# ghazalehnt/RecBole

Hardware: AMD Instinct MI355X
Metric: train positives/sec (+neg) per node (higher is better)
Workload: dtype fp32; 1 GPU; C2 BPR-MF ml-20m-shape: 138,494 users x 26,745 items (incl. PAD), ~20M interactions RO_RS 0.8/0.1/0.1, embedding 128, 4 uniform negatives, 512 positives (2,048 rows) per step, dense Adam; global_batch=512, per_gpu_batch=512, train_interactions=16014928, parallelism=single, exchange_graph=True, sampler=walk (bit-exact)

## Files before the change

include/mirec.h:

```cpp
#ifndef MIREC_H
#define MIREC_H

#include <stddef.h>
#include <stdint.h>

#ifdef __cplusplus
extern "C" {
#endif

#define MIREC_ABI_VERSION 19

int mirec_abi_version(void);
const char* mirec_last_error(void);

size_t mirec_sample_walk_workspace_size(int64_t batch_keys, int64_t num);
int mirec_sample_walk(const int32_t* random_list, int64_t L, int64_t* pr_dev,
                      const int64_t* keys, int64_t n_keys, int64_t batch_keys,
                      int64_t n_batches, int64_t num,
                      const int64_t* used_ptr, const int32_t* used_cols,
                      const uint32_t* used_bits, int64_t n_bits,
                      int64_t n_key_space, int reject,
                      int64_t* out, int64_t out_stride, int32_t* status_dev,
                      void* ws, size_t ws_bytes, void* stream);

// ... 202 lines not shown

int mirec_adam_multi_f32(const mirec_adam_table* tables, int32_t n_tables, int32_t d,
                         const float* step_consts_dev, const int32_t* step_base_dev,
                         int32_t step_off, double beta1, double beta2, double eps,
                         double weight_decay, void* stream);

#define MIREC_ADAM_ZERO_STATE 0x7fffffff
int mirec_adam_deferred_f32(const mirec_adam_table* tables, int32_t n_tables,
                            const int64_t* n_max_uniq, int32_t d,
                            const float* step_consts_dev, const int32_t* step_base_dev,
                            int32_t step_off, double beta1, double beta2, double eps,
                            double weight_decay, void* stream);
int mirec_adam_deferred_pair_f32(const mirec_adam_table* tables, const int64_t* n_max_uniq,
                                 int32_t d, const float* step_consts_dev,
                                 const int32_t* step_base_dev, int32_t step_off, double beta1,
                                 double beta2, double eps, double weight_decay, void* stream);

int mirec_adam_flush_f32(const mirec_adam_table* tables, int32_t n_tables, int32_t d,
                         const float* step_consts_dev, const int32_t* step_base_dev,
                         int32_t step_off, double beta1, double beta2, double eps,
                         double weight_decay, void* stream);
int mirec_adam_flush_rows_f32(const mirec_adam_table* tables, int32_t n_tables, int32_t d,
                              const int32_t* rows_per_wave, const float* step_consts_dev,
                              const int32_t* step_base_dev, int32_t step_off, double beta1,
                              double beta2, double eps, double weight_decay, void* stream);
int mirec_adam_flush_masked_f32(const mirec_adam_table* tables, int32_t n_tables, int32_t d,
                                const uint32_t* const* masks, const int32_t* want,
                                const int32_t* rows_per_wave, int32_t walk_waves,
                                const float* step_consts_dev, const int32_t* step_base_dev,
                                int32_t step_off, double beta1, double beta2, double eps,
                                double weight_decay, void* stream);
int mirec_row_bitmap(const int64_t* keys, int64_t n_keys, int64_t n_rows, uint32_t* bitmap,
                     void* stream);
int mirec_bpr_adam_step_f32(const mirec_adam_table* tables, const int64_t* n_max_uniq,
                            int32_t d, const int64_t* items, int64_t Bc, int32_t T, float gamma,
                            float grad_scale, float* loss_k, const int32_t* u_rec,
                            const int32_t* u_crec, const int32_t* i_rec, const int32_t* i_crec,
                            float* u_part, int32_t* u_join, float* i_part, int32_t* i_join,
                            const float* step_consts_dev, const int32_t* step_base_dev,
                            int32_t step_off, double beta1, double beta2, double eps,
                            double weight_decay, void* stream);
int mirec_step_records(const int64_t* user_keys, const int64_t* item_keys, int64_t n_batches,
                       int64_t Bc, int32_t T, int64_t n_users, int64_t n_items,
                       const int32_t* u_perm, const int32_t* u_uniq, const int32_t* u_seg,
                       const int32_t* u_nu, const int32_t* i_perm, const int32_t* i_uniq,
                       const int32_t* i_seg, const int32_t* i_nu, int32_t* u_rec,
                       int32_t* u_crec, int32_t* i_rec, int32_t* i_crec, int32_t* u_ahead,
                       int32_t* u_nah, int32_t* i_ahead, int32_t* i_nah, void* stream);
int64_t mirec_step_record_ints(int64_t per);

int mirec_copy_many(const void* const* src, void* const* dst, const int64_t* bytes, int n,
                    void* stream);

int mirec_write_bytes(void* dst_dev, const void* src_host, size_t n_bytes, void* stream);

int mirec_selftest_adam_math(uint64_t sqrt_stride, uint64_t n_div, uint64_t seed,
                             unsigned long long* out4_dev, void* stream);

int mirec_step_finish(const float* loss_k, int64_t n, float denom, float* loss_hist,
                      int32_t* step_idx_dev, void* stream);

int mirec_chunk_finish(const float* loss_k, int64_t n, int64_t stride, int32_t n_steps,
                       float denom, float* loss_hist, int32_t* step_base_dev,
                       int32_t* ticket_dev, void* stream);

int mirec_fullsort_topk_f32(const float* Uq, int64_t nq, const float* EI, int64_t I,
// ... 243 lines not shown
```

recbole_amd/_native.py:

```python
from __future__ import annotations

import ctypes
import os
from ctypes import c_double, c_float, c_int, c_int32, c_int64, c_size_t, c_void_p, c_char_p

import torch

_HERE = os.path.dirname(os.path.abspath(__file__))
LIB_PATH = os.environ.get("MIREC_LIB", os.path.join(_HERE, "_lib", "libmirec.so"))

_P = c_void_p


class RowsRef(ctypes.Structure):
    _fields_ = [('lo', _P), ('hi', _P), ('split', c_int64)]


class SpmmEpilogue(ctypes.Structure):
    _fields_ = [('add', RowsRef), ('add_scale', c_float), ('y', RowsRef), ('acc_in', RowsRef),
                ('acc_out', RowsRef), ('acc_scale', c_float)]


class CtxField(ctypes.Structure):
    _fields_ = [('kind', c_int32), ('seq_len', c_int32), ('ids', _P), ('vals', _P),
# ... 138 lines not shown
    "mirec_segment_reduce2_f32": (c_int, [_P, c_int32, _P, _P, _P, _P, _P, c_int64, _P, _P, _P,
                                          c_size_t, _P]),
    "mirec_segment_reduce2_pos_seg_f32": (c_int, [_P, c_int32, _P, _P, _P, _P, _P, _P, c_int64,
                                                  _P, _P, _P, c_size_t, _P]),
    "mirec_segment_scatter_add_workspace_size": (c_size_t, [c_int64, c_int32]),
    "mirec_segment_scatter_add_f32": (c_int, [_P, c_int32, _P, _P, _P, _P, c_int64, _P,
                                              c_int64, _P, c_size_t, _P]),
    "mirec_adam_sparse_grad_f32": (c_int, [_P, _P, _P, c_int64, c_int32, _P, _P, _P, _P, _P,
                                           c_int64, _P, _P, _P, c_double, c_double, c_double,
                                           c_double, _P]),
    "mirec_adam_flat_multi_f32": (c_int, [ctypes.POINTER(FlatParam), c_int32, _P, _P, c_double,
                                          c_double, c_double, c_double, _P]),
    "mirec_adam_flat_multi_advance_f32": (c_int, [ctypes.POINTER(FlatParam), c_int32, _P, _P, _P,
                                                  c_double, c_double, c_double, c_double, _P]),
    "mirec_adam_flat_f32": (c_int, [_P, _P, _P, c_int64, _P, _P, _P, c_double, c_double,
                                    c_double, c_double, _P]),
    "mirec_adam_multi_f32": (c_int, [ctypes.POINTER(AdamTable), c_int32, c_int32, _P, _P,
                                     c_int32, c_double, c_double, c_double, c_double, _P]),
    "mirec_adam_deferred_f32": (c_int, [ctypes.POINTER(AdamTable), c_int32, _P, c_int32, _P,
                                        _P, c_int32, c_double, c_double, c_double, c_double,
                                        _P]),
    "mirec_adam_deferred_pair_f32": (c_int, [ctypes.POINTER(AdamTable), _P, c_int32, _P, _P,
                                             c_int32, c_double, c_double, c_double, c_double,
                                             _P]),
    "mirec_adam_flush_f32": (c_int, [ctypes.POINTER(AdamTable), c_int32, c_int32, _P, _P,
                                     c_int32, c_double, c_double, c_double, c_double, _P]),
    "mirec_adam_flush_rows_f32": (c_int, [ctypes.POINTER(AdamTable), c_int32, c_int32, _P, _P,
                                          _P, c_int32, c_double, c_double, c_double, c_double,
                                          _P]),
    "mirec_adam_flush_masked_f32": (c_int, [ctypes.POINTER(AdamTable), c_int32, c_int32, _P, _P,
                                            _P, c_int32, _P, _P, c_int32, c_double, c_double,
                                            c_double, c_double, _P]),
    "mirec_row_bitmap": (c_int, [_P, c_int64, c_int64, _P, _P]),
    "mirec_bpr_adam_step_f32": (c_int, [ctypes.POINTER(AdamTable), _P, c_int32, _P, c_int64,
                                        c_int32, ctypes.c_float, ctypes.c_float, _P, _P, _P,
                                        _P, _P, _P, _P, _P, _P, _P, _P, c_int32, c_double,
                                        c_double, c_double, c_double, _P]),
    "mirec_step_record_ints": (c_int64, [c_int64]),
    "mirec_colsum_multi_f32": (c_int, [_P, _P, _P, _P, c_int32, _P]),
    "mirec_offset_keys": (c_int, [_P, _P, c_int32, c_int64, _P, _P]),
    "mirec_bpr_fwd_bwd_at_ids_f32": (c_int, [_P, c_int64, c_int32, _P, _P, _P, c_int64, c_int32,
                                             ctypes.c_float, ctypes.c_float, _P, _P, _P]),
    "mirec_chunk_group_fits": (c_int, [c_int64, c_int32, c_int64, c_int64, c_int32]),
    "mirec_chunk_group": (c_int, [_P, _P, c_int64, c_int64, c_int32, c_int64, c_int64] + [_P] * 16
                          + [_P]),
    "mirec_step_records": (c_int, [_P, _P, c_int64, c_int64, c_int32, c_int64, c_int64, _P, _P,
                                   _P, _P, _P, _P, _P, _P, _P, _P, _P, _P, _P, _P, _P, _P,
                                   _P]),
    "mirec_step_finish": (c_int, [_P, c_int64, c_float, _P, _P, _P]),
    "mirec_chunk_finish": (c_int, [_P, c_int64, c_int64, c_int32, c_float, _P, _P, _P, _P]),
    "mirec_fullsort_topk_f32": (c_int, [_P, c_int64, _P, c_int64, c_int32, _P, _P, _P, _P,
                                        c_int32, _P, _P, _P, _P]),
    "mirec_fullsort_topk_split_workspace_size": (ctypes.c_size_t, [c_int64, c_int32, c_int32]),
    "mirec_fullsort_topk_split_f32": (c_int, [_P, c_int64, _P, c_int64, c_int32, _P, _P, _P, _P,
                                              c_int32, c_int32, _P, ctypes.c_size_t, _P, _P, _P,
                                              _P]),
    "mirec_score_matrix_f32": (c_int, [_P, c_int64, _P, c_int64, c_int32, _P, _P]),
    "mirec_spmm_csr_f32": (c_int, [_P, _P, _P, c_int64, c_int32, _P, _P, _P, c_int64, c_int32,
                                   _P, _P, c_int64, _P, ctypes.POINTER(RowsRef),
                                   ctypes.POINTER(SpmmEpilogue), _P]),
    "mirec_ctx_fm_work_floats": (c_size_t, [c_int64, c_int32, c_int32]),
    "mirec_ctx_fm_fwd_f32": (c_int, [_P, c_int32, c_int64, c_int32, _P, _P, _P, _P, _P]),
    "mirec_ctx_fm_bwd_f32": (c_int, [_P, c_int32, c_int64, c_int32, _P, _P, _P, _P, _P]),
    "mirec_sigmoid_bce_mean_f32": (c_int, [_P, _P, _P, c_int64, c_float, _P, _P, _P, _P]),
    "mirec_sigmoid_bce_f32": (c_int, [_P, _P, _P, c_int64, c_float, _P, _P, _P, _P]),
    "mirec_colsum_f32": (c_int, [_P, c_int64, c_int64, _P, _P]),
# ... 91 lines not shown
```

recbole_amd/csrc/adam.hip:

```cpp

#include "adam_core.h"

namespace mirec {

template <int D>
__global__ __launch_bounds__(kAdamThreads) void adam_multi_kernel(
    const AdamTables tabs, const float* __restrict__ consts, const int32_t* __restrict__ step_base,
    int step_off, AdamConsts k) {
  constexpr int VPR = D / 4;
  constexpr int RPP = kAdamThreads / VPR;
  static_assert(kAdamThreads % VPR == 0, "row width");
  __shared__ int32_t slot[kAdamRows];
  __shared__ int32_t s_range[2];

  const int si = segment_of(tabs, blockIdx.x);
  const mirec_adam_table& T = tabs.t[si];
  float* __restrict__ P = T.p;
  float* __restrict__ M = T.m;
  float* __restrict__ V = T.v;
  const int32_t* __restrict__ uniq = T.uniq;

  const int64_t lo = ((int64_t)blockIdx.x - tabs.block_start[si]) * kAdamRows;
  const int64_t hi = min(T.n_rows, lo + kAdamRows);
  if (threadIdx.x < kAdamRows) slot[threadIdx.x] = -1;
// ... 208 lines not shown
  const uint32_t* bits[kMaxTables];
  int32_t want[kMaxTables];
};

__device__ __forceinline__ bool mask_selects(const uint32_t* __restrict__ bits, int want,
                                             int64_t r) {
  return !bits || (int)((bits[r >> 5] >> (r & 31)) & 1u) == want;
}

template <int D, bool MASKED>
__global__ __launch_bounds__(kAdamThreads) void adam_flush_scan_kernel(
    const AdamTables tabs, const float* __restrict__ consts, const int32_t* __restrict__ step_base,
    int step_off, AdamConsts k, FlushRows rows_per_wave, FlushMasks masks) {
  const int si = segment_of(tabs, blockIdx.x);
  const mirec_adam_table& T = tabs.t[si];
  const int R = rows_per_wave.r[si];
  const int lane = threadIdx.x & 63;
  const int64_t r0 =
      (((int64_t)blockIdx.x - tabs.block_start[si]) * (kAdamThreads / 64) + (threadIdx.x >> 6)) * R;
  if (r0 >= T.n_rows) return;
  const int target = step_base[0] + step_off;
  int raw = kZeroState;
  if (lane < R && r0 + lane < T.n_rows &&
      (!MASKED || mask_selects(masks.bits[si], masks.want[si], r0 + lane)))
    raw = T.last[r0 + lane];
  uint64_t todo = __ballot(flush_needs(T, raw, target));
  while (todo) {
    const int i = __builtin_ctzll(todo);
    todo &= todo - 1;
    flush_row<D>(T, r0 + i, __shfl(raw, i, 64), target, lane, consts, k);
  }
}

constexpr int kWalkRows = 32;

template <int D>
__global__ __launch_bounds__(64) void adam_flush_walk_kernel(
    const AdamTables tabs, const float* __restrict__ consts, const int32_t* __restrict__ step_base,
    int step_off, AdamConsts k, FlushMasks masks) {
  const int lane = threadIdx.x;
  const int target = step_base[0] + step_off;
  for (int si = 0; si < tabs.n_seg; ++si) {
    const mirec_adam_table& T = tabs.t[si];
    const uint32_t* __restrict__ bits = masks.bits[si];
    const uint32_t flip = masks.want[si] ? 0u : ~0u;
    const int64_t groups = (T.n_rows + kWalkRows - 1) / kWalkRows;
    for (int64_t g = blockIdx.x; g < groups; g += gridDim.x) {
      const int64_t r0 = g * kWalkRows;
      const uint32_t sel = bits ? (bits[g] ^ flip) : ~0u;
      int raw = kZeroState;
      if (lane < kWalkRows && r0 + lane < T.n_rows && ((sel >> lane) & 1u))
        raw = T.last[r0 + lane];
      uint64_t todo = __ballot(flush_needs(T, raw, target));
      while (todo) {
        const int i = __builtin_ctzll(todo);
        todo &= todo - 1;
        flush_row<D>(T, r0 + i, __shfl(raw, i, 64), target, lane, consts, k);
      }
    }
  }
}

}

using namespace mirec;

namespace {

enum class Sched { kStreamed, kDeferred, kFlush, kDeferredPair };

int launch_adam(Sched sched, const mirec_adam_table* tables, int32_t n_tables,
                const int64_t* n_max_uniq, int32_t d, const float* consts,
                const int32_t* step_base, int32_t step_off, double beta1, double beta2,
                double eps, double weight_decay, void* stream, const char* what,
                const int32_t* flush_rows = nullptr, const FlushMasks* masks = nullptr,
                int walk_waves = 0) {
  if (n_tables < 1 || n_tables > kMaxTables || !tables || !consts || !step_base) {
    set_error("%s: bad arguments (n_tables=%d)", what, n_tables);
    return -1;
  }
  if (((uintptr_t)consts & 15) != 0) {
    set_error("%s: step constants must be 16-byte aligned", what);
    return -1;
  }
  if (d != 4 && d != 16 && d != 32 && d != 64 && d != 128 && d != 256 &&
      !(d == 1 && sched != Sched::kStreamed)) {
    set_error("%s: row width %d not in {4,16,32,64,128,256} (1: deferred / flush)", what, d);
    return -1;
  }
  const int VPR = d / 4;
  const bool pair = sched == Sched::kDeferredPair;
  if (pair) {
    if (n_tables != 2 || d == 1) {
      set_error("%s: a pair is two tables, the first of width d > 1 (got %d tables, d=%d)",
                what, n_tables, d);
      return -1;
    }
    sched = Sched::kDeferred;
  }
  FlushRows fr;
  bool scan = false;
  for (int q = 0; q < kMaxTables; ++q) fr.r[q] = 1;
  if (sched == Sched::kFlush && flush_rows) {
    if (d < 64) {
      set_error("%s: rows per wave need d >= 64", what);
      return -1;
    }
    for (int q = 0; q < n_tables; ++q) {
      if (flush_rows[q] < 1 || flush_rows[q] > 64) {
        set_error("%s: rows per wave %d of table %d not in [1, 64]", what, flush_rows[q], q);
        return -1;
      }
      fr.r[q] = flush_rows[q];
    }
    scan = true;
  }
  const bool walk = masks && walk_waves > 0;
  if (masks && (sched != Sched::kFlush || d < 64 || (!scan && !walk))) {
    set_error("%s: a masked flush needs d >= 64 and rows per wave or a wave count", what);
    return -1;
  }
  FlushMasks fm;
  memset(&fm, 0, sizeof(fm));
  if (masks) fm = *masks;
  AdamTables tabs;
  memset(&tabs, 0, sizeof(tabs));
  const bool deferred = sched == Sched::kDeferred;
  tabs.n_seg = deferred ? 2 * n_tables : n_tables;
  int dvec = 1;
  if (deferred && n_max_uniq && d >= 4) {
    int64_t waves = 0;
    for (int q = 0; q < (pair ? 1 : n_tables); ++q)
      if (n_max_uniq[q] > 0)
        waves += n_max_uniq[q] * (tables[q].ahead_uniq ? 2 : 1) * ((d + 63) / 64);
    if (waves > 16 * 1024) dvec = 2;
    bool ahead = false;
    for (int q = 0; q < n_tables; ++q) ahead = ahead || tables[q].ahead_uniq != nullptr;
    if (dvec == 2 && d >= 128 && !ahead && !pair) dvec = 4;
  }
  int64_t blocks = 0;
  for (int q = 0; q < n_tables; ++q) {
    const mirec_adam_table& t = tables[q];
    const bool grouped = t.n_uniq != nullptr;
    if (!t.p || !t.m || !t.v || t.n_rows < 0 ||
        (grouped && (!t.uniq || !t.seg || !t.perm || !t.rows)) ||
        (sched != Sched::kStreamed && !t.last) ||
        (deferred && (!grouped || t.dense_grad || !n_max_uniq || n_max_uniq[q] < 0)) ||
        (deferred && (t.ahead_uniq == nullptr) != (t.ahead_n_uniq == nullptr))) {
      set_error("%s: bad table %d", what, q);
      return -1;
    }
    if (t.p_alt && (sched == Sched::kStreamed || d < 64 || pair)) {
      set_error("%s: table %d: parity buffer (p_alt) needs the deferred schedule and d >= 64",
                what, q);
      return -1;
    }
    tabs.t[q] = t;
// ... 19 lines not shown
  }
  (void)VPR;
  for (int q = tabs.n_seg; q <= 2 * kMaxTables; ++q) tabs.block_start[q] = blocks;
  if (blocks == 0) return 0;
  AdamConsts k;
  k.omb1 = (float)(1.0 - beta1);
  k.omb1m1 = k.omb1 - 1.0f;
  k.lerp_small = fabsf(k.omb1) < 0.5f;
  k.b2 = (float)beta2;
  k.omb2 = (float)(1.0 - beta2);
  k.eps = (float)eps;
  k.wd = (float)weight_decay;
  const dim3 grd((unsigned)blocks), blk(kAdamThreads);
  hipStream_t st = (hipStream_t)stream;
#define MIREC_ADAM_SCHED(DD)                                                                 \
  case DD:                                                                                   \
    if (sched == Sched::kStreamed)                                                           \
      hipLaunchKernelGGL(adam_multi_kernel<DD>, grd, blk, 0, st, tabs, consts, step_base,    \
                         step_off, k);                                                       \
    else if (deferred && pair)                                                               \
      hipLaunchKernelGGL((dvec == 2 ? adam_deferred_pair_kernel<DD, float2>                  \
                                    : adam_deferred_pair_kernel<DD, float>),                 \
                         grd, dim3(deferred_block(1)), 0, st, tabs, consts, step_base,       \
                         step_off, k);                                                       \
    else if (deferred)                                                                       \
      hipLaunchKernelGGL((dvec == 4 ? adam_deferred_kernel<DD, float4>                       \
                          : dvec == 2 ? adam_deferred_kernel<DD, float2>                     \
                                      : adam_deferred_kernel<DD, float>),                    \
                         grd, dim3(deferred_block(DD / dvec)), 0, st, tabs, consts,          \
                         step_base, step_off, k);                                            \
    else if (DD >= 64 && walk)                                                               \
      hipLaunchKernelGGL(adam_flush_walk_kernel<(DD >= 64 ? DD : 64)>, grd, dim3(64), 0, st,   \
                         tabs, consts, step_base, step_off, k, fm);                          \
    else if (DD >= 64 && scan && masks)                                                      \
      hipLaunchKernelGGL((adam_flush_scan_kernel<(DD >= 64 ? DD : 64), true>), grd, blk, 0,    \
                         st, tabs, consts, step_base, step_off, k, fr, fm);                  \
    else if (DD >= 64 && scan)                                                               \
      hipLaunchKernelGGL((adam_flush_scan_kernel<(DD >= 64 ? DD : 64), false>), grd, blk, 0,   \
                         st, tabs, consts, step_base, step_off, k, fr, fm);                  \
    else if (DD >= 64)                                                                       \
      hipLaunchKernelGGL(adam_flush_row_kernel<(DD >= 64 ? DD : 64)>, grd,                   \
                         dim3(kFlushRowThreads), 0, st, tabs,                                \
                         consts, step_base, step_off, k);                                    \
    else                                                                                     \
      hipLaunchKernelGGL(adam_flush_list_kernel<(DD < 64 ? DD : 16)>, grd, blk, 0, st, tabs, \
                         consts, step_base, step_off, k);                                    \
    break;
  switch (d) {
    case 1:
      if (deferred)
        hipLaunchKernelGGL((adam_deferred_kernel<1, float>), grd, dim3(deferred_block(1)), 0, st,
                           tabs, consts, step_base, step_off, k);
      else
        hipLaunchKernelGGL(adam_flush_list_kernel<1>, grd, blk, 0, st, tabs, consts, step_base,
                           step_off, k);
      break;
    MIREC_ADAM_SCHED(4)
    MIREC_ADAM_SCHED(16)
    MIREC_ADAM_SCHED(32)
    MIREC_ADAM_SCHED(64)
    MIREC_ADAM_SCHED(128)
    MIREC_ADAM_SCHED(256)
  }
#undef MIREC_ADAM_SCHED
  return launch_status(what);
}
// ... 73 lines not shown
                                           const int32_t* step_base_dev, int32_t step_off,
                                           double beta1, double beta2, double eps,
                                           double weight_decay, void* stream) {
  const char* what = "mirec_adam_flush_masked_f32";
  if (!tables || n_tables < 1 || n_tables > kMaxTables || !want || walk_waves < 0 ||
      walk_waves > 65536 || (walk_waves == 0) != (rows_per_wave != nullptr)) {
    set_error("%s: bad arguments (rows per wave for the scan form, or a wave count in "
              "[1, 65536] for the walk form)", what);
    return -1;
  }
  mirec_adam_table sel[kMaxTables];
  int32_t rows[kMaxTables];
  FlushMasks fm;
  memset(&fm, 0, sizeof(fm));
  int n = 0;
  for (int q = 0; q < n_tables; ++q) {
    if (want[q] < 0) continue;
    if (want[q] > 1) {
      set_error("%s: want[%d] = %d not in {-1, 0, 1}", what, q, want[q]);
      return -1;
    }
    sel[n] = tables[q];
    rows[n] = rows_per_wave ? rows_per_wave[q] : 1;
    fm.bits[n] = masks ? masks[q] : nullptr;
    fm.want[n] = want[q];
    ++n;
  }
  if (n == 0) return 0;
  return launch_adam(Sched::kFlush, sel, n, nullptr, d, step_consts_dev, step_base_dev, step_off,
                     beta1, beta2, eps, weight_decay, stream, what,
                     rows_per_wave ? rows : nullptr, &fm, walk_waves);
}

extern "C" int mirec_adam_sparse_grad_f32(float* p, float* m, float* v, int64_t n_rows,
                                          int32_t d, const float* rows, const int32_t* perm,
                                          const int32_t* uniq, const int32_t* seg,
                                          const int32_t* n_uniq_dev, int64_t n_max_uniq,
                                          const float* dense_grad, const float* step_consts_dev,
                                          const int32_t* step_idx_dev, double beta1,
                                          double beta2, double eps, double weight_decay,
                                          void* stream) {
  (void)n_max_uniq;
  if (n_rows == 0) return 0;
  mirec_adam_table t;
  memset(&t, 0, sizeof(t));
  t.p = p; t.m = m; t.v = v; t.n_rows = n_rows;
  t.rows = rows; t.perm = perm; t.uniq = uniq; t.seg = seg; t.n_uniq = n_uniq_dev;
  t.dense_grad = dense_grad;
  return mirec_adam_multi_f32(&t, 1, d, step_consts_dev, step_idx_dev, 0, beta1, beta2, eps,
                              weight_decay, stream);
}

namespace mirec {

__global__ __launch_bounds__(kAdamThreads) void adam_flat_kernel(
    float* __restrict__ p, float* __restrict__ m, float* __restrict__ v, int64_t n,
    const float* __restrict__ g, const float* __restrict__ consts,
    const int32_t* __restrict__ step_idx, AdamConsts k) {
  const StepConsts sc = step_consts(consts, step_idx[0]);
  for (int64_t i = (int64_t)blockIdx.x * blockDim.x + threadIdx.x; i < n;
       i += (int64_t)gridDim.x * blockDim.x) {
    float pp = p[i], mm = m[i], vv = v[i];
    adam_elem(pp, mm, vv, g[i], sc, k);
    p[i] = pp;
    m[i] = mm;
    v[i] = vv;
// ... 134 lines not shown
```

recbole_amd/csrc/step.hip:

```cpp
#include "adam_core.h"
#include "bpr_math.h"
#include "ahead.h"

namespace mirec {

struct StepLaunch {
  mirec_adam_table t[2];
  const int32_t* rec[2];
  const int32_t* crec[2];
  float* part[2];
  int32_t* join[2];
  int64_t block_start[7];
  int32_t seg_rows[6];
};

__device__ __forceinline__ int64_t clamp_id(int64_t id, int64_t n) {
  return id < 0 ? 0 : (id >= n ? n - 1 : id);
}


constexpr int kRecInts = 8;
constexpr int kRecInline = 2;
constexpr int kRowRec = 4 + kRecInline * kRecInts;
constexpr int kShare = kRecInline;
// ... 668 lines not shown
  return launch_status("mirec_step_records");
}

extern "C" int64_t mirec_step_record_ints(int64_t per) { return per < 0 ? -1 : rec_ints(per); }

namespace mirec {
__global__ __launch_bounds__(256) void row_bitmap_kernel(const int64_t* __restrict__ keys,
                                                         int64_t n_keys, int64_t n_rows,
                                                         uint32_t* __restrict__ bitmap) {
  const int64_t i = (int64_t)blockIdx.x * blockDim.x + threadIdx.x;
  if (i >= n_keys) return;
  const int64_t r = clamp_id(keys[i], n_rows);
  atomicOr(bitmap + (r >> 5), 1u << (r & 31));
}
}

extern "C" int mirec_row_bitmap(const int64_t* keys, int64_t n_keys, int64_t n_rows,
                                uint32_t* bitmap, void* stream) {
  const char* what = "mirec_row_bitmap";
  if (n_keys < 0 || n_rows <= 0 || !bitmap || (n_keys > 0 && !keys) ||
      n_keys > (int64_t)INT32_MAX * 256) {
    set_error("%s: bad arguments", what);
    return -1;
  }
  hipStream_t st = (hipStream_t)stream;
  const int rc = hip_status(hipMemsetAsync(bitmap, 0, (size_t)((n_rows + 31) / 32) * 4, st), what);
  if (rc) return rc;
  if (n_keys == 0) return 0;
  hipLaunchKernelGGL(row_bitmap_kernel, dim3((unsigned)((n_keys + 255) / 256)), dim3(256), 0, st,
                     keys, n_keys, n_rows, bitmap);
  return launch_status(what);
}

#if defined(MIREC_STEP_COUNT)
extern "C" int mirec_work_counters(unsigned long long* dst, int clear) {
  if (hipMemcpyFromSymbol(dst, HIP_SYMBOL(g_work), sizeof(g_work)) != hipSuccess) return -1;
  if (clear) {
    unsigned long long z[16] = {0};
    if (hipMemcpyToSymbol(HIP_SYMBOL(g_work), z, sizeof(z)) != hipSuccess) return -1;
  }
  return 0;
}
#endif

namespace mirec {
static int bits_for(int64_t n) {
  int b = 0;
  while (b < 40 && ((int64_t)1 << b) < n) ++b;
  return b;
}
}

namespace mirec {
static bool chunk_group_fits(int64_t Bc, int32_t T, int64_t n_users, int64_t n_items,
                             bool ahead) {
  if (Bc <= 0 || T < 1 || n_users <= 0 || n_items <= 0) return false;
  const int64_t KI = (int64_t)(1 + T) * Bc;
  const int pu = bits_for(Bc), pi = bits_for(KI);
  return !(Bc > kGrpUserMax || KI > kGrpMax || bits_for(n_users) + pu > 32 ||
           bits_for(n_items) + pi > 32 ||
           (ahead && (n_users > 32 * (int64_t)kGrpBitmapWords ||
                      n_items > 32 * (int64_t)kGrpBitmapWords)));
}
}

extern "C" int mirec_chunk_group_fits(int64_t Bc, int32_t T, int64_t n_users, int64_t n_items,
// ... 115 lines not shown
```

recbole_amd/trainer/chunk_plan.py:

```python
from __future__ import annotations

import bisect
import math


def plan_chunks(n, Bg, C, ramp, cuts=(), ramps=(0,)):
    full = n // Bg
    bounds = sorted({0, full} | {int(c) for c in cuts if 0 < int(c) < full})
    ramp_at = {int(r) for r in ramps}
    out = []
    for lo, hi in zip(bounds[:-1], bounds[1:]):
        ri = 0 if lo in ramp_at else len(ramp)
        b0 = lo
        while b0 < hi:
            size = ramp[ri] if ri < len(ramp) else C
            ri += 1
            nb = min(size, C, hi - b0)
            out.append((b0, nb, Bg))
            b0 += nb
    if n % Bg:
        out.append((full, 1, n % Bg))
    return out


# ... 15 lines not shown
    for i, (b0, nb, _) in enumerate(plan):
        entry = since > 0
        since += nb
        nxt_full = i + 1 < len(plan) and plan[i + 1][2] == Bg
        nxt_nb = plan[i + 1][1] if i + 1 < len(plan) else 0
        flush = (since >= flush_every or since + nxt_nb > flush_every * 3 // 2
                 or not nxt_full or b0 + nb in flush_at)
        if flush:
            since = 0
        flags.append((entry, flush_rows(b0 + nb, Bg, times, adam_mode, d, n_rows, busy0,
                                        max_rows) if flush else False))
    return flags


def bg_flush_chunks(plan, flags, Bg, adam_mode, fused_step, use_graph, min_steps=1,
                    enabled=True):
    on = bool(enabled and fused_step and use_graph and adam_mode == 'deferred')
    return [bool(on and flush and not entry and Bc == Bg and nb >= min_steps)
            for (_, nb, Bc), (entry, flush) in zip(plan, flags)]


def bg_flush_now(planned, c0, c1, nb, graph_ready, timed_kernels):
    return bool(planned and c0 == 0 and c1 == nb and graph_ready and not timed_kernels)


def masked_flush_rows(flush, nb, Bg, n_users, max_rows):
    frac = min(1.0, nb * Bg / max(n_users, 1))
    r = 1
    while r * 2 <= max_rows and r * 2 * frac <= 1.0:
        r *= 2
    return (r,) + tuple(flush[1:])


def chunk_of(plan, b):
    return max(bisect.bisect_right(plan, (b, math.inf)) - 1, 0)
```

recbole_amd/trainer/fused.py:

```python
from __future__ import annotations

import ctypes
import math
import os
from types import SimpleNamespace

import numpy as np
import torch

from recbole_amd import ops
from recbole_amd._native import AdamTable, ChunkPrep, check, lib
from recbole_amd.trainer import chunk_plan
from recbole_amd.trainer.exchange import ExchangeLayout

REC_CONTRIB = 8
ADAM_MODES = ('deferred', 'streamed')


_PREP_STREAMS = {}


def _prep_streams_for(dev, n=2):
    key = (str(dev), n)
    got = _PREP_STREAMS.get(key)
# ... 22 lines not shown
                break
        torch.cuda.synchronize(dev)
        (chosen if free else spare).append(cand)
    while len(chosen) < n:
        chosen.append(spare.pop(0) if spare else torch.cuda.Stream(device=dev))
    _PREP_STREAMS[key] = chosen
    return chosen


class _Lists(object):

    def __init__(self, C, per, dev, ahead):
        i32 = dict(dtype=torch.int32, device=dev)
        self.perm, self.uniq = torch.empty(C * per, **i32), torch.empty(C * per, **i32)
        self.seg, self.nu = torch.empty(C * (per + 1), **i32), torch.zeros(C, **i32)
        self.ahead = torch.empty(C * per, **i32) if ahead else None
        self.nah = torch.zeros(C, **i32) if ahead else None


class _Slot(object):

    def __init__(self, C, B, T, G, dev, ahead, tab=None):
        Bg = G * B
        KI = (1 + T) * Bg
        self.user_keys = torch.empty(C * Bg, dtype=torch.int64, device=dev)
        self.item_keys = torch.empty(C * KI, dtype=torch.int64, device=dev)
        self.lu = self.li = None
        if G > 1:
            self.lu = torch.empty(C * B, dtype=torch.int64, device=dev)
            self.li = torch.empty(C * (1 + T) * B, dtype=torch.int64, device=dev)
        self.tab = tab or [_Lists(C, per, dev, ahead) for per in (Bg, KI)]
        self.records = None
        self.bitmap = None
        self.bg_done = None
        self.bg_busy = False
        self.prep = None
        self.ready, self.walked, self.free = (torch.cuda.Event() for _ in range(3))
        cur = torch.cuda.current_stream(dev)
        for ev in (self.ready, self.walked, self.free):
            ev.record(cur)
        self.free_recorded = False
        self.group_pending = False
        self.ready_on_model = False
        self.chunk = None
        self.graphs = {}


class FusedBPRTrainStep(object):

    CHUNK = 64
    SLOTS = 3
    RAMP = (8, 16, 32)
    FLUSH_EVERY = 64
    FLUSH_SPARSE_MAX_ROWS = 8
    MAIN_FIRST = os.environ.get('MIREC_MAIN_FIRST', '1') != '0'
    SPEC_WALK = os.environ.get('MIREC_SPEC_WALK', '1') != '0'
    BG_FLUSH = os.environ.get('MIREC_BG_FLUSH', '1') != '0'
    BG_WAVES = int(os.environ.get('MIREC_BG_WAVES', '1536'))
    BG_MIN_STEPS = 32

    def __init__(self, model, optimizer, train_data, chunk=None, use_graph=True,
                 adam_mode='deferred', dist=None, fused_step=None):
        if adam_mode not in ADAM_MODES:
            raise ValueError(f'adam_mode must be one of {ADAM_MODES}, got {adam_mode!r}')
        self.model = model
        self.opt = optimizer
        self.data = train_data
        (self.pU, self.nU), (self.pI, self.nI) = model.fused_embedding_tables()
        self.device = self.pU.device
        self.B = train_data.step
        self.times = train_data.times
        self.uid_field = train_data.uid_field
        self.iid_field = train_data.iid_field
        self.C = chunk or self.CHUNK
        self.use_graph = use_graph
        self.adam_mode = adam_mode
        self.group = dist
        if dist is not None:
            import torch.distributed as tdist
            self.G, self.rank = tdist.get_world_size(dist), tdist.get_rank(dist)
            if str(tdist.get_backend(dist)) != 'nccl':
                self.use_graph = False
        else:
            self.G, self.rank = 1, 0
        B, T, G, d = self.B, self.times, self.G, self.pU.shape[1]
        self.Bg = G * B
        self.d = d
        dev = self.device
        deferred = adam_mode == 'deferred'
        applies = deferred and G == 1 and d in (64, 128, 256)
        if fused_step and not applies:
            raise ValueError('fused_step needs adam_mode="deferred", one rank and d in '
                             '{64, 128, 256}')
        self.fused_step = applies if fused_step is None else bool(fused_step)
        self.loss_k = torch.empty(self.C * self.Bg, dtype=torch.float32, device=dev)
        self.samp_ws = torch.empty(lib().mirec_sample_walk_workspace_size(self.Bg, T),
                                   dtype=torch.uint8, device=dev)
        self.sort_ws = None
        side = _prep_streams_for(dev, 3 if self.fused_step else 2)
        self.prep_stream, self.group_stream = side[:2]
        self.bg_stream = side[2] if self.fused_step else None
        self.zero_i32 = torch.zeros(1, dtype=torch.int32, device=dev)
        self.loss_hist = torch.zeros(1, dtype=torch.float32, device=dev)
        self.consts = torch.zeros(4, dtype=torch.float32, device=dev)
        self.step_idx = torch.zeros(1, dtype=torch.int32, device=dev)
        self.ticket = torch.zeros(1, dtype=torch.int32, device=dev)
        self.kernel_events = None
        self.kernel_uniq = []
        self.n_eager_steps = 0
        self._rec_w = {}
        self._spec_buf = self._spec_stats = None
        self._gs_R = self._gs = None
        self._users = self._items = None
        self.n_batches = 0
        self._plan, self._flags, self._flush_at = [], [], set()
        self._bg = []
        self._bg_pending = None
        self._bg_mark = torch.cuda.Event()
        self._bg_mark.record(torch.cuda.current_stream(dev))
        self._busy0 = None
        self._batches_enqueued = 0
        self._current = True
        self._next_chunk = self._next_group = self._prep_limit = 0
        self._cur = None
        self._last_walked = None
        self._deferred_waits = []
        self._urgent = False
        self._late_top_up = None
        self.opt._ensure_state(self.pU)
        self.opt._ensure_state(self.pI)
        self._tables = (AdamTable * 2)()
        g = self.opt.param_groups[0]
        self._adam_args = (g['betas'][0], g['betas'][1], g['eps'], g['weight_decay'])
        self._allocate()

    def _allocate(self):
        B, T, G, d, dev = self.B, self.times, self.G, self.d, self.device
        deferred = self.adam_mode == 'deferred'
        self.layout = ExchangeLayout(G, B, T, d)
        self.xbuf = torch.empty(self.Bg * (2 + T) * d, dtype=torch.float32, device=dev)
        self.xchg = torch.empty(G * self.layout.W, dtype=torch.float32, device=dev)
        self.slots = [_Slot(self.C, B, T, G, dev, deferred) for _ in range(self.SLOTS)]
        self.lastU = self.lastI = None
        if deferred:
            self.lastU = torch.zeros(self.nU, dtype=torch.int32, device=dev)
            self.lastI = torch.zeros(self.nI, dtype=torch.int32, device=dev)
        self.pU_alt = torch.empty_like(self.pU.data) if self.fused_step else None
        self.pI_alt = torch.empty_like(self.pI.data) if self.fused_step else None
        self._step_scratch = None
        if self.fused_step:
            for sl in self.slots:
                sl.records = [torch.empty(self.C * w, dtype=torch.int32, device=dev)
                              for w in self._rec_ints(self.Bg)]
                sl.bitmap = torch.zeros((self.nU + 31) // 32, dtype=torch.int32, device=dev)
                sl.bg_done = torch.cuda.Event()
                sl.bg_done.record(torch.cuda.current_stream(dev))
            self._step_scratch = ops.step_scratch(self.Bg, T, d, dev)
        self._n_max = (ctypes.c_int64 * 2)(self.Bg, (1 + T) * self.Bg)
        self._fill_tables()

    def _flush_rows(self, b_end):
        return chunk_plan.flush_rows(b_end, self.Bg, self.times, self.adam_mode, self.d,
                                     [t.n_rows for t in self._tables], self._busy0,
                                     self.FLUSH_SPARSE_MAX_ROWS)

    def _chunk_of(self, b):
        return chunk_plan.chunk_of(self._plan, b)

    def _dp_slice(self, Bc):
        return self.G > 1 and Bc == self.Bg

    def _prepare(self, slot, chunk, on=None):
        if slot.free_recorded and on is None and not slot.free.query():
            self.prep_stream.wait_event(slot.free)
        if slot.bg_busy:
            (on if on is not None else self.prep_stream).wait_event(slot.bg_done)
            slot.bg_busy = False
        if self._dp_slice(chunk[2]):
            self._prepare_dp(slot, chunk)
        else:
            self._prepare_native(slot, chunk, on)

    def _prepare_native(self, slot, chunk, on):
        b0, nb, Bc = chunk
        cp = self._chunk_prep(slot)
        cp.users, cp.items = self._users.data_ptr(), self._items.data_ptr()
        cp.s0, cp.n_batches, cp.Bc = b0 * self.Bg, nb, Bc
# ... 44 lines not shown
        KI = (1 + T) * Bc
        with torch.cuda.stream(self.prep_stream):
            users, items = self._copy_keys_and_walk(slot, chunk)
            for l, keys, per, n in zip(slot.tab, (users, items), (Bc, KI), (self.nU, self.nI)):
                self.sort_ws = ops.segment_sort_batched(keys, per, n, l.perm, l.uniq, l.seg,
                                                        l.nu, ws=self.sort_ws)
            lay, g, B = self.layout, self.rank, self.B
            slot.lu[:nb * B].view(nb, B).copy_(lay.local_users(users, g))
            slot.li[:nb * (1 + T) * B].view(nb, 1 + T, B).copy_(lay.local_items(items, g))
            if self.adam_mode == 'deferred':
                for l, per in zip(slot.tab, (Bc, KI)):
                    ops.uniq_ahead_diff(l.uniq, l.nu, per, nb, l.ahead, l.nah)
            slot.ready.record(self.prep_stream)
        slot.chunk = chunk

    def _apply_deferred_waits(self):
        for st, ev in self._deferred_waits:
            st.wait_event(ev)
        self._deferred_waits = []

    def _prepare_group(self, slot):
        self._apply_deferred_waits()
        self.group_stream.wait_event(slot.walked)
        self._group_on(slot, self.group_stream)

    def _group_on(self, slot, st):
        check(lib().mirec_prepare_chunk_group(ctypes.byref(slot.prep), st.cuda_stream),
              'mirec_prepare_chunk_group')
        b0, nb, Bc = slot.chunk
        if slot.bitmap is not None and self._bg[self._chunk_of(b0)]:
            check(lib().mirec_row_bitmap(slot.user_keys.data_ptr(), nb * Bc, self.nU,
                                         slot.bitmap.data_ptr(), st.cuda_stream),
                  'mirec_row_bitmap')
        slot.ready.record(st)
        slot.group_pending = False

    def _chunk_prep(self, slot):
        if slot.prep is not None:
            return slot.prep
        dev = self.device
        with torch.cuda.stream(self.prep_stream):
            walk = self.data.sampler.walk_args(dev)
        rl, pr, up, uc, bits, n_bits, reject, status = walk
        T = self.times
        nsort = lib().mirec_segment_sort_workspace_size(self.C * (1 + T) * self.Bg, self.nI)
        if self.sort_ws is None or self.sort_ws.numel() < nsort:
            self.sort_ws = torch.empty(nsort, dtype=torch.uint8, device=dev)
        p = lambda x: x.data_ptr() if x is not None else None
        cp = ChunkPrep()
        cp.T = T
        cp.user_keys, cp.item_keys = slot.user_keys.data_ptr(), slot.item_keys.data_ptr()
        cp.random_list, cp.L, cp.pr_dev = rl.data_ptr(), rl.numel(), pr.data_ptr()
        cp.used_ptr, cp.used_cols = (p(up), p(uc)) if bits is None else (None, None)
        cp.used_bits, cp.n_bits = p(bits), n_bits if bits is not None else 0
        cp.n_users, cp.n_items, cp.reject, cp.status = self.nU, self.nI, int(reject), p(status)
        cp.walk_ws, cp.walk_ws_bytes = self.samp_ws.data_ptr(), self.samp_ws.numel()
        cp.sort_ws, cp.sort_ws_bytes = self.sort_ws.data_ptr(), self.sort_ws.numel()
        for tag, l in zip('ui', slot.tab):
            for f, x in (('perm', l.perm), ('uniq', l.uniq), ('seg', l.seg), ('nu', l.nu),
                         ('ahead', l.ahead), ('nah', l.nah)):
                if x is not None:
                    setattr(cp, f'{tag}_{f}', x.data_ptr())
        if slot.records is not None:
            cp.u_rec, cp.u_crec, cp.i_rec, cp.i_crec = (r.data_ptr() for r in slot.records)
        spec = self._spec_ws()
        if spec is not None:
# ... 161 lines not shown
    def _flush_background(self, slot, t_end, stream):
        bg = self.bg_stream
        self._bg_mark.record(stream)
        bg.wait_event(self._bg_mark)
        bg.wait_event(slot.ready)
        check(lib().mirec_adam_flush_masked_f32(
            self._tables, 2, self.d, (ctypes.c_void_p * 2)(slot.bitmap.data_ptr(), None),
            (ctypes.c_int32 * 2)(0, -1), None, int(self.BG_WAVES), self.consts.data_ptr(),
            self.zero_i32.data_ptr(), int(t_end), *self._adam_args, bg.cuda_stream),
            'mirec_adam_flush_masked_f32')
        slot.bg_done.record(bg)
        slot.bg_busy = True
        self._bg_pending = slot.bg_done

    def _await_background(self, stream):
        if self._bg_pending is not None:
            stream.wait_event(self._bg_pending)
            self._bg_pending = None

    def _entry_lists(self, slot):
        return [(l.uniq, l.nu) for l in slot.tab]

    def _entry(self, slot, stream):
        if self.adam_mode != 'deferred':
            return
        t = (AdamTable * 2)()
        ctypes.memmove(t, self._tables, ctypes.sizeof(t))
        self._point_tables(t, [SimpleNamespace(perm=uniq, uniq=uniq, seg=uniq, nu=self.zero_i32,
                                               ahead=uniq, nah=n)
                               for uniq, n in self._entry_lists(slot)], 0, (0, 0), True)
        t[0].rows = t[1].rows = self.xbuf.data_ptr()
        self._adam(stream, -1, t, 'ahead')

    def _grad_scale(self, Bc):
        R = Bc * self.times
        if self._gs_R != R:
            self._gs_R = R
            self._gs = float(np.float32(1.0) / np.float32(R))
        return self._gs

    def _graph_for(self, slot, nb, entry, flush, masked=False):
        key = (nb, entry, flush, masked)
        g = slot.graphs.get(key)
        if g is None:
            g = torch.cuda.CUDAGraph()
            cap = torch.cuda.Stream(device=self.device)
            cap.wait_stream(torch.cuda.current_stream(self.device))
            with torch.cuda.graph(g, stream=cap):
                if entry:
                    self._entry(slot, cap)
                for c in range(nb):
                    self._step(slot, c, self.Bg, cap, c, c + 1 < nb)
                self._finish(0, nb, self.Bg, cap)
                if flush and masked:
                    self._flush_masked(cap, slot, chunk_plan.masked_flush_rows(
                        flush, nb, self.Bg, self.nU, self.FLUSH_SPARSE_MAX_ROWS))
                elif flush:
                    self._flush(cap, flush)
            torch.cuda.current_stream(self.device).wait_stream(cap)
            slot.graphs[key] = g
        return g

    def _capture_variants(self):
        S = len(self.slots)
        variants = sorted({(k % S, n, e, f, bg) for k, ((_, n, Bc), (e, f), bg) in
                           enumerate(zip(self._plan, self._flags, self._bg)) if Bc == self.Bg},
                          key=lambda v: (v[0], v[1], v[2], repr(v[3]), v[4]))
        for k, n, e, f, bg in variants:
            self._graph_for(self.slots[k], n, e, f, bg)

    def begin_epoch(self, cuts=(), hold_prep_from=None, flush_at=()):
        self._await_background(torch.cuda.current_stream(self.device))
        data = self.data
        if data.shuffle:
            data._shuffle()
        inter = data.dataset.inter_feat
        self._users = inter[self.uid_field]
        self._items = inter[self.iid_field]
        if not self._users.is_cuda:
            raise RuntimeError('fused train step needs the train table on the GPU')
        self.n_batches = nb = math.ceil(self._users.numel() / self.Bg)
        table = self.opt.step_constants(self.opt.n_steps + 1, max(nb, 1)).reshape(-1)
        ptrs = [(t.p, t.m, t.v) for t in self._tables]
        self._fill_tables()
        stale = ptrs != [(t.p, t.m, t.v) for t in self._tables]
        if self.consts.numel() < table.size:
            self.consts = torch.zeros(table.size, dtype=torch.float32, device=self.device)
            self.loss_hist = torch.zeros(max(nb, 1), dtype=torch.float32, device=self.device)
            stale = True
        if stale:
            self._drop_graphs()
        self.consts[:table.size].copy_(torch.from_numpy(table))
        self.loss_hist.zero_()
        self.step_idx.zero_()
        n_rows = [t.n_rows for t in self._tables]
        self._busy0 = n_rows
        self._batches_enqueued = 0
        if self.adam_mode == 'deferred':
            busy = []
            for m, v, last in self._adam_state():
                ops.zero_state_marks(m, v, last, self._adam_args[3])
                busy.append((last != ops.ADAM_ZERO_STATE).sum())
            self._busy0 = [int(x) for x in torch.stack(busy).cpu()]
        if self.fused_step:
            self.pU_alt.copy_(self.pU.data)
            self.pI_alt.copy_(self.pI.data)
        ramps = (0,) if hold_prep_from is None else (0, int(hold_prep_from))
        self._plan = chunk_plan.plan_chunks(self._users.numel(), self.Bg, self.C, self.RAMP,
                                            cuts, ramps)
        self._flush_at = set(int(b) for b in flush_at)
        self._flags = chunk_plan.chunk_flags(self._plan, self.Bg, self.FLUSH_EVERY,
                                             self._flush_at, self.times, self.adam_mode, self.d,
                                             n_rows, self._busy0, self.FLUSH_SPARSE_MAX_ROWS)
        self._bg = chunk_plan.bg_flush_chunks(self._plan, self._flags, self.Bg, self.adam_mode,
                                              self.fused_step, self.use_graph,
                                              self.BG_MIN_STEPS, self.BG_FLUSH)
        if self.use_graph:
            self._capture_variants()
        self.prep_stream.wait_stream(torch.cuda.current_stream(self.device))
        self._last_walked = None
        self._deferred_waits, self._urgent, self._late_top_up = [], False, None
        self._next_chunk = 0
        self._next_group = 0
        self._prep_limit = (len(self._plan) if hold_prep_from is None
                            else self._chunk_of(hold_prep_from))
        self._cur = None
        for s in self.slots:
            s.free_recorded = False
            if not self._dp_slice(self.Bg):
                self._chunk_prep(s)
        for _ in range(len(self.slots)):
            self._issue_prep()
        self._issue_groups(len(self.slots))
        return nb

    def release_prep(self, upto=None):
        self._prep_limit = (len(self._plan) if upto is None
                            else self._chunk_of(max(int(upto) - 1, 0)) + 1)
        if self._next_chunk < min(len(self._plan), self._prep_limit):
            k = self._next_chunk
            if self.MAIN_FIRST and not self._dp_slice(self._plan[k][2]):
                self._issue_prep(on=torch.cuda.current_stream(self.device))
                self._late_top_up = k
            else:
                self._issue_prep()

    def _issue_prep(self, on=None):
        k = self._next_chunk
        if k >= min(len(self._plan), self._prep_limit):
# ... 17 lines not shown
        if self._cur is not None:
            prev = self.slots[self._cur % S]
            prev.free.record(stream)
            prev.free_recorded = True
        if (self.MAIN_FIRST and self._next_chunk == k and k < min(len(self._plan), self._prep_limit)
                and not self._dp_slice(self._plan[k][2])):
            self._issue_prep(on=stream)
            self._late_top_up = k
        while self._next_chunk <= k and self._next_chunk < min(len(self._plan),
                                                               self._prep_limit):
            self._issue_prep()
        if self._next_chunk <= k:
            raise RuntimeError(f'chunk {k} is held (begin_epoch(hold_prep_from=...)): '
                               'call release_prep() first')
        self._issue_groups(k + 1)
        slot = self.slots[k % S]
        if self._late_top_up != k:
            self._top_up_prep(k)
        if not slot.ready_on_model:
            stream.wait_event(slot.ready)
        self._cur = k

    def run_batches(self, b_start, b_end):
        stream = torch.cuda.current_stream(self.device)
        b = b_start
        while b < b_end:
            k = self._chunk_of(b)
            b0, nb, Bc = self._plan[k]
            entry, flush = self._flags[k]
            self._await_background(stream)
            self._enter_chunk(k, stream)
            slot = self.slots[k % len(self.slots)]
            c0, c1 = b - b0, min(nb, b_end - b0)
            key = (nb, entry, flush, self._bg[k])
            if (self.use_graph and c0 == 0 and c1 == nb and Bc == self.Bg
                    and self.kernel_events is None and key in slot.graphs):
                if chunk_plan.bg_flush_now(self._bg[k], c0, c1, nb, key in slot.graphs,
                                           self.kernel_events is not None):
                    self._flush_background(slot, b0 + nb, stream)
                slot.graphs[key].replay()
                self._current = flush
            else:
                self.n_eager_steps += c1 - c0
                if c0 == 0 and entry:
                    self._entry(slot, stream)
                for c in range(c0, c1):
                    self._step(slot, c, Bc, stream, 0, c + 1 < nb)
                    self._finish(c, 1, Bc, stream)
                self._current = False
                if c1 == nb and flush:
                    self._flush(stream, flush)
                    self._current = True
            if self._late_top_up == k:
                self._late_top_up = None
                self._urgent = True
                self._top_up_prep(k)
                self._urgent = False
            self._issue_groups(k + len(self.slots))
            b = b0 + c1
            self._batches_enqueued = b

    def _top_up_prep(self, k):
        lim = min(len(self._plan), self._prep_limit, k + len(self.slots))
        while self._next_chunk < lim:
            self._issue_prep()

    def sync_params(self):
        self._await_background(torch.cuda.current_stream(self.device))
        if not self._current:
# ... 37 lines not shown
```

Baseline: 26.76 million positives/s.

## Advance lazy Adam rows to their first-read step at chunk entry

During chunk prep, a new kernel records for each user and item row the first step in the chunk that reads it (atomicMin over the per-step unique lists). At chunk entry, a new flush kernel brings only those rows' deferred Adam state up to that step, replacing the full entry pass inside the captured graph. The aim is to skip catch-up work for rows the chunk never touches and move it out of the per-step path. The cost is an extra prep kernel, a memset per table and more graph variants.

```diff
diff --git a/include/mirec.h b/include/mirec.h
--- a/include/mirec.h
+++ b/include/mirec.h
@@ -258,6 +258,14 @@
                                 double weight_decay, void* stream);
 int mirec_row_bitmap(const int64_t* keys, int64_t n_keys, int64_t n_rows, uint32_t* bitmap,
                      void* stream);
+#define MIREC_FIRST_NOT_READ (-1)
+int mirec_first_read(const int32_t* uniq, const int32_t* n_uniq, int64_t n_batches, int64_t per,
+                     int64_t n_rows, int32_t* first, void* stream);
+int mirec_adam_flush_first_f32(const mirec_adam_table* tables, int32_t n_tables, int32_t d,
+                               const int32_t* const* first, const int32_t* rows_per_wave,
+                               const float* step_consts_dev, const int32_t* step_base_dev,
+                               int32_t step_off, double beta1, double beta2, double eps,
+                               double weight_decay, void* stream);
 int mirec_bpr_adam_step_f32(const mirec_adam_table* tables, const int64_t* n_max_uniq,
                             int32_t d, const int64_t* items, int64_t Bc, int32_t T, float gamma,
                             float grad_scale, float* loss_k, const int32_t* u_rec,
diff --git a/recbole_amd/_native.py b/recbole_amd/_native.py
--- a/recbole_amd/_native.py
+++ b/recbole_amd/_native.py
@@ -194,6 +194,10 @@
                                             _P, c_int32, _P, _P, c_int32, c_double, c_double,
                                             c_double, c_double, _P]),
     "mirec_row_bitmap": (c_int, [_P, c_int64, c_int64, _P, _P]),
+    "mirec_first_read": (c_int, [_P, _P, c_int64, c_int64, c_int64, _P, _P]),
+    "mirec_adam_flush_first_f32": (c_int, [ctypes.POINTER(AdamTable), c_int32, c_int32, _P, _P,
+                                           _P, _P, c_int32, c_double, c_double, c_double,
+                                           c_double, _P]),
     "mirec_bpr_adam_step_f32": (c_int, [ctypes.POINTER(AdamTable), _P, c_int32, _P, c_int64,
                                         c_int32, ctypes.c_float, ctypes.c_float, _P, _P, _P,
                                         _P, _P, _P, _P, _P, _P, _P, _P, c_int32, c_double,
diff --git a/recbole_amd/csrc/adam.hip b/recbole_amd/csrc/adam.hip
--- a/recbole_amd/csrc/adam.hip
+++ b/recbole_amd/csrc/adam.hip
@@ -264,6 +264,40 @@
   }
 }
 
+struct FlushFirst {
+  const int32_t* first[kMaxTables];
+};
+constexpr int kFirstNotRead = MIREC_FIRST_NOT_READ;
+
+template <int D>
+__global__ __launch_bounds__(kAdamThreads) void adam_flush_first_kernel(
+    const AdamTables tabs, const float* __restrict__ consts, const int32_t* __restrict__ step_base,
+    int step_off, AdamConsts k, FlushRows rows_per_wave, FlushFirst ff) {
+  const int si = segment_of(tabs, blockIdx.x);
+  const mirec_adam_table& T = tabs.t[si];
+  const int R = rows_per_wave.r[si];
+  const int lane = threadIdx.x & 63;
+  const int64_t r0 =
+      (((int64_t)blockIdx.x - tabs.block_start[si]) * (kAdamThreads / 64) + (threadIdx.x >> 6)) * R;
+  if (r0 >= T.n_rows) return;
+  const int base = step_base[0] + step_off;
+  int raw = kZeroState, target = 0;
+  if (lane < R && r0 + lane < T.n_rows) {
+    const int f = ff.first[si][r0 + lane];
+    if (f > kFirstNotRead) {
+      target = base + f;
+      raw = T.last[r0 + lane];
+    }
+  }
+  uint64_t todo = __ballot(min(raw, target) < target);
+  while (todo) {
+    const int i = __builtin_ctzll(todo);
+    todo &= todo - 1;
+    flush_row<D>(T, r0 + i, __builtin_amdgcn_readfirstlane(__shfl(raw, i, 64)),
+                 __builtin_amdgcn_readfirstlane(__shfl(target, i, 64)), lane, consts, k);
+  }
+}
+
 constexpr int kWalkRows = 32;
 
 template <int D>
@@ -306,7 +340,7 @@
                 const int32_t* step_base, int32_t step_off, double beta1, double beta2,
                 double eps, double weight_decay, void* stream, const char* what,
                 const int32_t* flush_rows = nullptr, const FlushMasks* masks = nullptr,
-                int walk_waves = 0) {
+                int walk_waves = 0, const FlushFirst* firsts = nullptr) {
   if (n_tables < 1 || n_tables > kMaxTables || !tables || !consts || !step_base) {
     set_error("%s: bad arguments (n_tables=%d)", what, n_tables);
     return -1;
@@ -355,6 +389,13 @@
   FlushMasks fm;
   memset(&fm, 0, sizeof(fm));
   if (masks) fm = *masks;
+  if (firsts && (sched != Sched::kFlush || !scan || masks)) {
+    set_error("%s: per-row targets need the flush with rows per wave and no mask", what);
+    return -1;
+  }
+  FlushFirst ff;
+  memset(&ff, 0, sizeof(ff));
+  if (firsts) ff = *firsts;
   AdamTables tabs;
   memset(&tabs, 0, sizeof(tabs));
   const bool deferred = sched == Sched::kDeferred;
@@ -440,6 +481,9 @@
     else if (DD >= 64 && walk)                                                               \
       hipLaunchKernelGGL(adam_flush_walk_kernel<(DD >= 64 ? DD : 64)>, grd, dim3(64), 0, st,   \
                          tabs, consts, step_base, step_off, k, fm);                          \
+    else if (DD >= 64 && scan && firsts)                                                     \
+      hipLaunchKernelGGL(adam_flush_first_kernel<(DD >= 64 ? DD : 64)>, grd, blk, 0, st, tabs, \
+                         consts, step_base, step_off, k, fr, ff);                            \
     else if (DD >= 64 && scan && masks)                                                      \
       hipLaunchKernelGGL((adam_flush_scan_kernel<(DD >= 64 ? DD : 64), true>), grd, blk, 0,    \
                          st, tabs, consts, step_base, step_off, k, fr, fm);                  \
@@ -579,6 +623,35 @@
                      rows_per_wave ? rows : nullptr, &fm, walk_waves);
 }
 
+extern "C" int mirec_adam_flush_first_f32(const mirec_adam_table* tables, int32_t n_tables,
+                                          int32_t d, const int32_t* const* first,
+                                          const int32_t* rows_per_wave,
+                                          const float* step_consts_dev,
+                                          const int32_t* step_base_dev, int32_t step_off,
+                                          double beta1, double beta2, double eps,
+                                          double weight_decay, void* stream) {
+  const char* what = "mirec_adam_flush_first_f32";
+  if (!tables || n_tables < 1 || n_tables > kMaxTables || !first || !rows_per_wave) {
+    set_error("%s: bad arguments (first-read arrays and rows per wave, per table)", what);
+    return -1;
+  }
+  mirec_adam_table sel[kMaxTables];
+  int32_t rows[kMaxTables];
+  FlushFirst ff;
+  memset(&ff, 0, sizeof(ff));
+  int n = 0;
+  for (int q = 0; q < n_tables; ++q) {
+    if (!first[q]) continue;
+    sel[n] = tables[q];
+    rows[n] = rows_per_wave[q];
+    ff.first[n] = first[q];
+    ++n;
+  }
+  if (n == 0) return 0;
+  return launch_adam(Sched::kFlush, sel, n, nullptr, d, step_consts_dev, step_base_dev, step_off,
+                     beta1, beta2, eps, weight_decay, stream, what, rows, nullptr, 0, &ff);
+}
+
 extern "C" int mirec_adam_sparse_grad_f32(float* p, float* m, float* v, int64_t n_rows,
                                           int32_t d, const float* rows, const int32_t* perm,
                                           const int32_t* uniq, const int32_t* seg,
diff --git a/recbole_amd/csrc/step.hip b/recbole_amd/csrc/step.hip
--- a/recbole_amd/csrc/step.hip
+++ b/recbole_amd/csrc/step.hip
@@ -724,6 +724,39 @@
   return launch_status(what);
 }
 
+namespace mirec {
+__global__ __launch_bounds__(256) void first_read_kernel(const int32_t* __restrict__ uniq,
+                                                         const int32_t* __restrict__ n_uniq,
+                                                         int64_t per, int64_t n_rows,
+                                                         uint32_t* __restrict__ first) {
+  const int c = blockIdx.y;
+  const int64_t i = (int64_t)blockIdx.x * blockDim.x + threadIdx.x;
+  if (i >= per || i >= n_uniq[c]) return;
+  const int64_t r = uniq[(int64_t)c * per + i];
+  if (r < 0 || r >= n_rows) return;
+  atomicMin(first + r, (uint32_t)c);
+}
+}
+
+extern "C" int mirec_first_read(const int32_t* uniq, const int32_t* n_uniq, int64_t n_batches,
+                                int64_t per, int64_t n_rows, int32_t* first, void* stream) {
+  const char* what = "mirec_first_read";
+  if (n_batches < 0 || n_batches > 32767 || per < 0 || per > INT32_MAX || n_rows <= 0 ||
+      !first || (n_batches > 0 && per > 0 && (!uniq || !n_uniq))) {
+    set_error("%s: bad arguments", what);
+    return -1;
+  }
+  hipStream_t st = (hipStream_t)stream;
+  static_assert(MIREC_FIRST_NOT_READ == -1, "reset by bytes of 0xff");
+  const int rc = hip_status(hipMemsetAsync(first, 0xff, (size_t)n_rows * 4, st), what);
+  if (rc) return rc;
+  if (n_batches == 0 || per == 0) return 0;
+  hipLaunchKernelGGL(first_read_kernel, dim3((unsigned)((per + 255) / 256), (unsigned)n_batches),
+                     dim3(256), 0, st, uniq, n_uniq, per, n_rows,
+                     reinterpret_cast<uint32_t*>(first));
+  return launch_status(what);
+}
+
 #if defined(MIREC_STEP_COUNT)
 extern "C" int mirec_work_counters(unsigned long long* dst, int clear) {
   if (hipMemcpyFromSymbol(dst, HIP_SYMBOL(g_work), sizeof(g_work)) != hipSuccess) return -1;
diff --git a/recbole_amd/trainer/chunk_plan.py b/recbole_amd/trainer/chunk_plan.py
--- a/recbole_amd/trainer/chunk_plan.py
+++ b/recbole_amd/trainer/chunk_plan.py
@@ -71,5 +71,21 @@
     return (r,) + tuple(flush[1:])
 
 
+def advance_chunks(plan, Bg, adam_mode, fused_step, use_graph, min_steps=1, enabled=True):
+    on = bool(enabled and fused_step and use_graph and adam_mode == 'deferred')
+    return [bool(on and Bc == Bg and nb >= min_steps) for _, nb, Bc in plan]
+
+
+def advance_rows(nb, Bg, times, n_rows, max_rows):
+    out = []
+    for per, rows in zip((Bg, (1 + times) * Bg), n_rows):
+        frac = min(1.0, nb * per / max(rows, 1))
+        r = 1
+        while r * 2 <= max_rows and r * 2 * frac <= 1.0:
+            r *= 2
+        out.append(r)
+    return tuple(out)
+
+
 def chunk_of(plan, b):
     return max(bisect.bisect_right(plan, (b, math.inf)) - 1, 0)
diff --git a/recbole_amd/trainer/fused.py b/recbole_amd/trainer/fused.py
--- a/recbole_amd/trainer/fused.py
+++ b/recbole_amd/trainer/fused.py
@@ -78,6 +78,7 @@
         self.tab = tab or [_Lists(C, per, dev, ahead) for per in (Bg, KI)]
         self.records = None
         self.bitmap = None
+        self.first = None
         self.bg_done = None
         self.bg_busy = False
         self.prep = None
@@ -104,6 +105,8 @@
     BG_FLUSH = os.environ.get('MIREC_BG_FLUSH', '1') != '0'
     BG_WAVES = int(os.environ.get('MIREC_BG_WAVES', '1536'))
     BG_MIN_STEPS = 32
+    CHUNK_ADVANCE = os.environ.get('MIREC_CHUNK_ADVANCE', '1') != '0'
+    ADV_MIN_STEPS = 32
 
     def __init__(self, model, optimizer, train_data, chunk=None, use_graph=True,
                  adam_mode='deferred', dist=None, fused_step=None):
@@ -161,6 +164,7 @@
         self.n_batches = 0
         self._plan, self._flags, self._flush_at = [], [], set()
         self._bg = []
+        self._adv = []
         self._bg_pending = None
         self._bg_mark = torch.cuda.Event()
         self._bg_mark.record(torch.cuda.current_stream(dev))
@@ -199,6 +203,8 @@
                 sl.records = [torch.empty(self.C * w, dtype=torch.int32, device=dev)
                               for w in self._rec_ints(self.Bg)]
                 sl.bitmap = torch.zeros((self.nU + 31) // 32, dtype=torch.int32, device=dev)
+                sl.first = [torch.full((n,), -1, dtype=torch.int32, device=dev)
+                            for n in (self.nU, self.nI)]
                 sl.bg_done = torch.cuda.Event()
                 sl.bg_done.record(torch.cuda.current_stream(dev))
             self._step_scratch = ops.step_scratch(self.Bg, T, d, dev)
@@ -309,6 +315,12 @@
             check(lib().mirec_row_bitmap(slot.user_keys.data_ptr(), nb * Bc, self.nU,
                                          slot.bitmap.data_ptr(), st.cuda_stream),
                   'mirec_row_bitmap')
+        if slot.first is not None and self._adv[self._chunk_of(b0)]:
+            for l, per, n, first in zip(slot.tab, (Bc, (1 + self.times) * Bc),
+                                        (self.nU, self.nI), slot.first):
+                check(lib().mirec_first_read(l.uniq.data_ptr(), l.nu.data_ptr(), nb, per, n,
+                                             first.data_ptr(), st.cuda_stream),
+                      'mirec_first_read')
         slot.ready.record(st)
         slot.group_pending = False
 
@@ -536,6 +548,13 @@
         t[0].rows = t[1].rows = self.xbuf.data_ptr()
         self._adam(stream, -1, t, 'ahead')
 
+    def _advance(self, slot, stream, nb):
+        rows = chunk_plan.advance_rows(nb, self.Bg, self.times, (self.nU, self.nI),
+                                       self.FLUSH_SPARSE_MAX_ROWS)
+        self._launch('advance', stream, 'mirec_adam_flush_first_f32', self._tables, 2, self.d,
+                     (ctypes.c_void_p * 2)(*[f.data_ptr() for f in slot.first]),
+                     (ctypes.c_int32 * 2)(*rows), *self._sched(0))
+
     def _grad_scale(self, Bc):
         R = Bc * self.times
         if self._gs_R != R:
@@ -543,15 +562,15 @@
             self._gs = float(np.float32(1.0) / np.float32(R))
         return self._gs
 
-    def _graph_for(self, slot, nb, entry, flush, masked=False):
-        key = (nb, entry, flush, masked)
+    def _graph_for(self, slot, nb, entry, flush, masked=False, advance=False):
+        key = (nb, entry, flush, masked, advance)
         g = slot.graphs.get(key)
         if g is None:
             g = torch.cuda.CUDAGraph()
             cap = torch.cuda.Stream(device=self.device)
             cap.wait_stream(torch.cuda.current_stream(self.device))
             with torch.cuda.graph(g, stream=cap):
-                if entry:
+                if entry and not advance:
                     self._entry(slot, cap)
                 for c in range(nb):
                     self._step(slot, c, self.Bg, cap, c, c + 1 < nb)
@@ -567,11 +586,12 @@
 
     def _capture_variants(self):
         S = len(self.slots)
-        variants = sorted({(k % S, n, e, f, bg) for k, ((_, n, Bc), (e, f), bg) in
-                           enumerate(zip(self._plan, self._flags, self._bg)) if Bc == self.Bg},
-                          key=lambda v: (v[0], v[1], v[2], repr(v[3]), v[4]))
-        for k, n, e, f, bg in variants:
-            self._graph_for(self.slots[k], n, e, f, bg)
+        variants = sorted({(k % S, n, e, f, bg, adv) for k, ((_, n, Bc), (e, f), bg, adv) in
+                           enumerate(zip(self._plan, self._flags, self._bg, self._adv))
+                           if Bc == self.Bg},
+                          key=lambda v: (v[0], v[1], v[2], repr(v[3]), v[4], v[5]))
+        for k, n, e, f, bg, adv in variants:
+            self._graph_for(self.slots[k], n, e, f, bg, adv)
 
     def begin_epoch(self, cuts=(), hold_prep_from=None, flush_at=()):
         self._await_background(torch.cuda.current_stream(self.device))
@@ -619,6 +639,9 @@
         self._bg = chunk_plan.bg_flush_chunks(self._plan, self._flags, self.Bg, self.adam_mode,
                                               self.fused_step, self.use_graph,
                                               self.BG_MIN_STEPS, self.BG_FLUSH)
+        self._adv = chunk_plan.advance_chunks(self._plan, self.Bg, self.adam_mode,
+                                              self.fused_step, self.use_graph,
+                                              self.ADV_MIN_STEPS, self.CHUNK_ADVANCE)
         if self.use_graph:
             self._capture_variants()
         self.prep_stream.wait_stream(torch.cuda.current_stream(self.device))
@@ -702,9 +725,11 @@
             self._enter_chunk(k, stream)
             slot = self.slots[k % len(self.slots)]
             c0, c1 = b - b0, min(nb, b_end - b0)
-            key = (nb, entry, flush, self._bg[k])
+            key = (nb, entry, flush, self._bg[k], self._adv[k])
             if (self.use_graph and c0 == 0 and c1 == nb and Bc == self.Bg
                     and self.kernel_events is None and key in slot.graphs):
+                if self._adv[k]:
+                    self._advance(slot, stream, nb)
                 if chunk_plan.bg_flush_now(self._bg[k], c0, c1, nb, key in slot.graphs,
                                            self.kernel_events is not None):
                     self._flush_background(slot, b0 + nb, stream)
```

Result: faster. 27.33 million positives/s (median of 6 runs) (+2.1%).
